# biagiom/spark-network-traffic-classifier

Hardware: NVIDIA H100
Metric: flow-records/sec fit+transform (higher is better)
Workload: dtype u8 bins / uint32 histograms / f64 split scoring (f32 records)

## Files before the change

### spark-network-traffic-classifier_b200/b200flow/forest.py

```python
import math
from dataclasses import dataclass

import numpy as np
import torch

from . import _lib
from ._lib import NODE_DTYPE, SPLIT_DTYPE, B200FlowError, UnsupportedParamError, call, ptr

import os as _os
CHUNK_ROWS = 2048
FUSED = True
TOP_LEVELS = int(_os.environ.get("B200FLOW_TOP_LEVELS", "8"))
DEDUP = True
_PIN = True
PROFILE = None


def _timed(name, fn, *args):
    if PROFILE is None:
        return call(fn, *args)
    e0, e1 = torch.cuda.Event(enable_timing=True), torch.cuda.Event(enable_timing=True)
    e0.record()
    call(fn, *args)
    e1.record()
# ... 552 lines not shown
    if U > 0:
        call("b200flow_bag_fill", ptr(W), T, U, ptr(blk_off), ptr(ent))
    del W, uid

    slot_tree = torch.arange(T, dtype=torch.int32, device=dev)
    slot_nid = torch.ones(T, dtype=torch.int32, device=dev)
    slot_node = torch.arange(T, dtype=torch.int32, device=dev)
    idx = torch.arange(T, dtype=torch.int64, device=dev) * nb
    seg_begin = blk_off[idx].contiguous()
    seg_end = blk_off[idx + nb].contiguous()
    n_slots = T
    level = 0
    per_slot_hist = m * n_bins * C * 4
    group_slots = max(1, HIST_BUDGET_BYTES // per_slot_hist)
    stats = dict(levels=0, slots=0, entries=0, hist_launches=0, rows=n, unique_rows=U)

    stats["route_chunk"], stats["route_passes"] = route_ch if fused else 0, route_passes if fused else 0
    stats["record_format"], stats["record_bytes"] = ("packed", rec_bytes) if field_desc is not None else ("bytes", stride)

    def chunk_table(nch):
        off = torch.empty(nch.shape[0] + 1, dtype=torch.int64, device=dev)
        call("b200flow_exclusive_scan_i32_to_i64", ptr(nch), nch.shape[0], ptr(off), ptr(total))
        return off, int(total.item())

    def level_subsets(ns, s_tree, s_nid):
        sub = torch.empty((ns, m), dtype=torch.int16, device=dev)
        call("b200flow_feature_subsets", seed, ns, ptr(s_tree), ptr(s_nid), F, m, ptr(sub))
        return sub

    def plan_route(ns, split_, begin_, end_, total_out, s_node=None, gain_out=None, cursors_=None):
        nch = torch.empty(ns, dtype=torch.int32, device=dev)
        call("b200flow_plan_route", ns, ptr(split_), ptr(begin_), ptr(end_), route_ch, ptr(s_node), ptr(gain_out), ptr(nch), ptr(cursors_))
        roff = torch.empty(ns + 1, dtype=torch.int64, device=dev)
        call("b200flow_exclusive_scan_i32_to_i64", ptr(nch), ns, ptr(roff), ptr(total_out))
        if PROFILE is not None:
            PROFILE.setdefault("_route_entries", []).append(torch.where(nch > 0, end_ - begin_, torch.zeros_like(end_)).sum())
        return roff

    route_chunks_max = E // route_ch + 1

    world = dist.get_world_size(group) if group is not None else 1
    rank = dist.get_rank(group) if group is not None else 0
    REC = 64 + 12 * C
    use_rs = world > 1 and bdist.is_nccl(group)

    def score_sharded(h_full, gs, sub, lvl, split_, nc_, lc_, rc_):
        K = int(max(1, min(RS_CHUNKS, gs, (gs * hsz * 4) // max(RS_MIN_BYTES, 1))))
        bounds = [gs * i // K for i in range(K + 1)]
        ev0 = None
        if PROFILE is not None:
            ev0 = torch.cuda.Event(enable_timing=True); ev0.record()
        jobs = []
        for k in range(K):
            s0, g = bounds[k], bounds[k + 1] - bounds[k]
            per = -(-g // world)
            mine = torch.empty(per * hsz, dtype=torch.int32, device=dev)
            w = dist.reduce_scatter_tensor(mine, h_full[s0 * hsz:(s0 + world * per) * hsz], group=group, async_op=True)
            jobs.append((s0, g, per, mine, w))
        gathers = []
        for s0, g, per, mine, w in jobs:
            w.wait()
            lo = rank * per
            cnt = max(0, min(per, g - lo))
            local = torch.empty(per * REC, dtype=torch.uint8, device=dev)
            sec = [local[:per * 64], local[per * 64:per * (64 + 4 * C)], local[per * (64 + 4 * C):per * (64 + 8 * C)], local[per * (64 + 8 * C):]]
            if cnt > 0:
                _timed("score_level", "b200flow_score_level", ptr(mine), cnt, ptr(sub[s0 + lo:s0 + lo + cnt]), m, n_bins, C, ptr(feat_bins),
                       ptr(feat_kind), lvl, p.max_depth, int(p.min_instances_per_node), float(p.min_info_gain), ptr(sec[0]), ptr(sec[1]),
                       ptr(sec[2]), ptr(sec[3]))
            gathered = torch.empty((world, per * REC), dtype=torch.uint8, device=dev)
            gw = dist.all_gather_into_tensor(gathered, local, group=group, async_op=True)
            gathers.append((s0, per, gathered, gw))
        for s0, per, gathered, gw in gathers:
            gw.wait()
            o = 0
            for dst, width in ((split_, 64), (nc_.view(torch.uint8), 4 * C), (lc_.view(torch.uint8), 4 * C), (rc_.view(torch.uint8), 4 * C)):
                dst.view(-1)[s0 * width:(s0 + world * per) * width].view(world, per * width).copy_(gathered[:, o:o + per * width])
                o += per * width
        if ev0 is not None:
            ev1 = torch.cuda.Event(enable_timing=True); ev1.record()
            PROFILE.setdefault("level_exchange", []).append((ev0, ev1))

    def run_route(roff, rch_dev, n_parents, split_, child_slot_, cursors_, next_subset_, n_next_cap, route=True):
        hist_next = torch.zeros((n_next_cap + world - 1) * hsz, dtype=torch.int32, device=dev)
        cmax = route_chunks_max + n_parents
        scratch = torch.empty(cmax * 4, dtype=torch.int32, device=dev)
        _timed("route_hist_level", "b200flow_route_hist_level", ptr(rec_tp), rec_stride, F, ptr(field_desc), ptr(ent), ptr(ent2), n_parents,
               ptr(seg_begin), ptr(seg_end), ptr(roff), ptr(rch_dev), cmax, route_ch, ptr(split_), ptr(child_slot_), ptr(cursors_),
               ptr(scratch), ptr(next_subset_), m, n_bins, C, ptr(hist_next), 1 if route else 0)
        _lib.launches += route_passes - 1
        stats["hist_launches"] += route_passes
        return hist_next

    side_stream = torch.cuda.Stream(device=dev)
    host_cnt = torch.empty(5, dtype=torch.int64).pin_memory() if _PIN else None
    subset = level_subsets(n_slots, slot_tree, slot_nid)
    hist_ready = None
    counters = None
    if fused and n_slots * hsz * 4 <= HIST_BUDGET_BYTES:
        pseudo = np.zeros(T, SPLIT_DTYPE); pseudo["bin_thr"] = 255; pseudo["flags"] = 4
        pseudo_t = _lib.h2d(pseudo.view(np.uint8).reshape(T, 64), dev)
        child0 = torch.stack([torch.arange(T, dtype=torch.int32, device=dev),
                              torch.full((T,), -1, dtype=torch.int32, device=dev)], 1).contiguous().view(-1)
        cursors0 = torch.zeros(2 * T, dtype=torch.int32, device=dev)
        roff0 = plan_route(T, pseudo_t, seg_begin, seg_end, total)
        hist_full = run_route(roff0, total, T, pseudo_t, child0, cursors0, subset, T, route=False)
        hist_ready = hist_full[:T * hsz]
    while n_slots > 0:
        grow_pool(pool_size + 2 * n_slots)
        lens = (seg_end - seg_begin) if hist_ready is None else None
        n_alloc = n_slots + world - 1
        split = torch.empty((n_alloc, 64), dtype=torch.uint8, device=dev)
        node_counts = torch.empty((n_alloc, C), dtype=torch.int32, device=dev)
        left_counts = torch.empty((n_alloc, C), dtype=torch.int32, device=dev)
        right_counts = torch.empty((n_alloc, C), dtype=torch.int32, device=dev)
        chunk_off = None
        if hist_ready is None:
            nch = ((lens + (CHUNK_ROWS - 1)) // CHUNK_ROWS).to(torch.int32).contiguous()
            chunk_off, n_chunks = chunk_table(nch)
        groups = [(0, n_slots)] if hist_ready is not None else \
            [(g0, min(n_slots, g0 + group_slots)) for g0 in range(0, n_slots, group_slots)]
        for g0, g1 in groups:
            gs = g1 - g0
            if hist_ready is not None:
                h = hist_ready
            else:
                h = torch.zeros(gs * hsz, dtype=torch.int32, device=dev)
                if g0 == 0 and g1 == n_slots:
                    coff, gch = chunk_off, n_chunks
                else:
                    coff = (chunk_off[g0:g1 + 1] - chunk_off[g0]).contiguous()
                    gch = int((chunk_off[g1] - chunk_off[g0]).item())
                _timed("hist_level", "b200flow_hist_level", ptr(tp), stride, F, ptr(ent), gs,
                       ptr(seg_begin[g0:g1]), ptr(seg_end[g0:g1]), ptr(coff), gch, CHUNK_ROWS, ptr(subset[g0:g1]), m, n_bins, C, ptr(h))
                stats["hist_launches"] += 1
                if PROFILE is not None:
                    PROFILE.setdefault("_hist_entries", []).append(lens[g0:g1].sum())
            if use_rs and hist_ready is not None and gs * hsz * 4 >= RS_MIN_BYTES:
                score_sharded(hist_full, gs, subset, level, split, node_counts, left_counts, right_counts)
                del h
                continue
            if group is not None:
                if PROFILE is not None:
                    ev0 = torch.cuda.Event(enable_timing=True); ev0.record()
                bdist.all_reduce_(h, group)
                if PROFILE is not None:
                    ev1 = torch.cuda.Event(enable_timing=True); ev1.record()
                    PROFILE.setdefault("level_exchange", []).append((ev0, ev1))
            _timed("score_level", "b200flow_score_level", ptr(h), gs, ptr(subset[g0:g1]), m, n_bins, C, ptr(feat_bins), ptr(feat_kind),
                   level, p.max_depth, int(p.min_instances_per_node), float(p.min_info_gain), ptr(split[g0:g1]),
                   ptr(node_counts[g0:g1]), ptr(left_counts[g0:g1]), ptr(right_counts[g0:g1]))
            del h
        split, node_counts, left_counts, right_counts = split[:n_slots], node_counts[:n_slots], left_counts[:n_slots], right_counts[:n_slots]
        hist_ready = None
        nblk = (n_slots + 255) // 256
        if counters is None or counters.numel() < 8 + nblk + 1:
            fresh = torch.zeros(8 + 2 * nblk + 1024, dtype=torch.int64, device=dev)
            if counters is None:
                fresh[0:1].fill_(pool_size)
            else:
                fresh[:8] = counters[:8]
            counters = fresh
        next_tree = torch.empty(2 * n_slots, dtype=torch.int32, device=dev)
        next_nid = torch.empty(2 * n_slots, dtype=torch.int32, device=dev)
        next_node = torch.empty(2 * n_slots, dtype=torch.int32, device=dev)
        next_parent = torch.empty(2 * n_slots, dtype=torch.int32, device=dev)
        child_slot = torch.empty(2 * n_slots, dtype=torch.int32, device=dev)
        _timed("grow_level", "b200flow_grow_level", n_slots, ptr(slot_tree), ptr(slot_nid), ptr(slot_node), ptr(split), ptr(node_counts),
# ... 96 lines not shown
```

### spark-network-traffic-classifier_b200/csrc/forest.cu

```cuda
#include <float.h>
#include <stdlib.h>
#include <string.h>

#include "common.cuh"

namespace b200flow {

constexpr int kMaxSubset = 128;

__global__ void __launch_bounds__(128) feature_subsets_kernel(uint64_t seed, int n_slots, const int32_t* __restrict__ slot_tree,
                                                              const uint32_t* __restrict__ slot_nid, int F, int m,
                                                              uint16_t* subset) {
    int s = blockIdx.x * blockDim.x + threadIdx.x;
    if (s >= n_slots) return;
    uint16_t* out = subset + (int64_t)s * m;
    if (m >= F) { for (int i = 0; i < F; ++i) out[i] = (uint16_t)i; return; }
    uint16_t pos[kMaxSubset], val[kMaxSubset], pick[kMaxSubset];
    int nt = 0;
    const int tree = slot_tree[s]; const uint32_t nid = slot_nid[s];
    uint4 r = make_uint4(0, 0, 0, 0);
    for (int i = 0; i < m; ++i) {
        if ((i & 3) == 0) r = philox_keyed(seed, PURPOSE_FEAT, (uint32_t)tree, nid, (uint32_t)(i >> 2), 0u);
        uint32_t w = (i & 3) == 0 ? r.x : (i & 3) == 1 ? r.y : (i & 3) == 2 ? r.z : r.w;
        int j = i + (int)(w % (uint32_t)(F - i));
// ... 391 lines not shown
    const uint8_t* __restrict__ tp, int stride, const b2f_entry* __restrict__ ent, b2f_entry* ent_out, int n_slots,
    const int64_t* __restrict__ seg_begin, const int64_t* __restrict__ seg_end, const int64_t* __restrict__ chunk_off,
    int chunk_rows, const b200flow_split* __restrict__ split, int32_t* cursors) {
    const int64_t c = blockIdx.x;
    const int s = find_slot(chunk_off, n_slots, c);
    const b200flow_split sp = split[s];
    if (sp.flags & 1) return;
    const bool keepL = !(sp.flags & 2), keepR = !(sp.flags & 4);
    if (!keepL && !keepR) return;
    const int64_t sb = seg_begin[s], se = seg_end[s];
    const int64_t b = sb + (c - chunk_off[s]) * chunk_rows;
    const int64_t e = min(se, b + chunk_rows);
    const int lane = lane_id();
    b2f_entry ents[kPartPerThread]; uint32_t dec = 0;
    int nL = 0, nR = 0;
#pragma unroll
    for (int k = 0; k < kPartPerThread; ++k) {
        const int64_t i = b + threadIdx.x + (int64_t)k * blockDim.x;
        int d = 0; ents[k] = make_uint2(0u, 0u);
        if (i < e) {
            ents[k] = ent[i];
            const int bin = tp[(int64_t)ents[k].x * stride + sp.feat];
            const bool left = sp.kind == 0 ? (bin <= sp.bin_thr) : ((sp.mask[bin >> 6] >> (bin & 63)) & 1ull);
            d = left ? (keepL ? 1 : 0) : (keepR ? 2 : 0);
        }
        dec |= (uint32_t)d << (2 * k);
        nL += __popc(__ballot_sync(0xffffffffu, d == 1));
        nR += __popc(__ballot_sync(0xffffffffu, d == 2));
    }
    int baseL = 0, baseR = 0;
    if (lane == 0) { if (nL) baseL = atomicAdd(&cursors[2 * s], nL); if (nR) baseR = atomicAdd(&cursors[2 * s + 1], nR); }
    baseL = __shfl_sync(0xffffffffu, baseL, 0); baseR = __shfl_sync(0xffffffffu, baseR, 0);
#pragma unroll
    for (int k = 0; k < kPartPerThread; ++k) {
        const int d = (dec >> (2 * k)) & 3;
        const uint32_t mL = __ballot_sync(0xffffffffu, d == 1), mR = __ballot_sync(0xffffffffu, d == 2);
        const uint32_t lt = (1u << lane) - 1u;
        if (d == 1) ent_out[sb + baseL + __popc(mL & lt)] = ents[k];
        else if (d == 2) ent_out[se - 1 - (baseR + __popc(mR & lt))] = ents[k];
        baseL += __popc(mL); baseR += __popc(mR);
    }
}

#ifndef B2F_EVICT_FIRST
#define B2F_EVICT_FIRST 1
#endif
#ifndef B2F_GRAN
#define B2F_GRAN 16
#endif
constexpr int kGran = B2F_GRAN;
__host__ __device__ inline int route_granules(int F) { return (F + 1 + kGran - 1) / kGran; }
__host__ __device__ inline int route_pitch(int F) { return kGran == 16 ? route_granules(F) : (route_granules(F) | 1); }
constexpr bool kEvictFirst = B2F_EVICT_FIRST != 0;

constexpr int kPackedMaxBytes = 64;
__device__ __forceinline__ int packed_swizzle_words(int i, int nq) {
    return nq == 2 ? ((i >> 2) & 1) << 2 : nq == 4 ? ((i >> 1) & 3) << 2 : 0;
}

struct RouteChunk { int32_t slot; int32_t n; long long begin; };

__global__ void route_chunks_kernel(const int64_t* __restrict__ chunk_off, int n_slots, const int64_t* __restrict__ n_chunks_dev,
                                    const int64_t* __restrict__ seg_begin, const int64_t* __restrict__ seg_end, int CH,
                                    RouteChunk* out) {
    int64_t c = (int64_t)blockIdx.x * blockDim.x + threadIdx.x;
    if (c >= *n_chunks_dev) return;
    const int s = find_slot(chunk_off, n_slots, c);
    RouteChunk rc; rc.slot = s; rc.begin = seg_begin[s] + (c - chunk_off[s]) * CH;
    rc.n = (int)(min(seg_end[s], (int64_t)rc.begin + CH) - rc.begin);
    out[c] = rc;
}

struct RouteArgs {
    const uint8_t* tp; int stride; int F;
    const int32_t* field_desc;
    const b2f_entry* ent; b2f_entry* ent_out;
    const RouteChunk* chunks; const int64_t* n_chunks_dev;
    const int64_t* seg_begin; const int64_t* seg_end;
    const b200flow_split* split; const int32_t* child_slot; int32_t* cursors;
    const uint16_t* subset_next; int m_total;
    int j0; int m;
    int n_bins; int C; uint32_t* hist_next;
    int route;
};

__host__ __device__ inline size_t route_tab_bytes(int mp, bool packed) { return packed && mp <= 12 ? (size_t)2 * mp * 32 * 8 : 0; }

template <int M, int NW, int KS, int MERGE, int NQ>
__global__ void __launch_bounds__(NW * 32, NW == 8 ? 3 : (NW == 16 ? 2 : 1)) route_hist_level_kernel(const RouteArgs a) {
    extern __shared__ __align__(16) uint32_t sm_u32[];
    constexpr bool PACKED = NQ > 0;
    constexpr bool kTab = PACKED && M > 0 && MERGE == 2;
    constexpr int kThreads = NW * 32, kSub = KS * 32;
    constexpr int gran = PACKED ? 16 : kGran;
    const int m = M > 0 ? M : a.m;
    const int F = a.F;
    const int tid = threadIdx.x, lane = lane_id(), wid = warp_id();
    const int nq = PACKED ? NQ : route_granules(F);
    const int rs = PACKED ? NQ * 16 : route_pitch(F) * kGran;
    const int nbC = a.n_bins * a.C, hsz = m * nbC;
    const int tile_words = rs * kSub / 4;
    uint32_t* tile = sm_u32 + (size_t)wid * tile_words;
    uint32_t* sh_hist = sm_u32 + (size_t)NW * tile_words;
    int* sh_fpos = (int*)(sh_hist + 2 * hsz);
    uint2* sh_tab = (uint2*)(sh_fpos + 2 * m);
    __shared__ b200flow_split sh_split;
    __shared__ int sh_child[2], sh_route_field;

    const int64_t n_chunks = *a.n_chunks_dev;
    const int64_t c0 = n_chunks * blockIdx.x / gridDim.x, c1 = n_chunks * (blockIdx.x + 1) / gridDim.x;
    if (c0 >= c1) return;
    auto flush = [&]() {
        for (int side = 0; side < 2; ++side) {
            const int cs = sh_child[side];
            if (cs < 0) continue;
            uint32_t* gh = a.hist_next + ((int64_t)cs * a.m_total + a.j0) * nbC;
            uint32_t* sh = sh_hist + side * hsz;
            for (int i = tid; i < hsz; i += kThreads) { const uint32_t v = sh[i]; if (v) { atomicAdd(gh + i, v); sh[i] = 0; } }
        }
    };
    for (int i = tid; i < 2 * hsz; i += kThreads) sh_hist[i] = 0;
    auto desc_at = [&](int64_t c) { return c < c1 ? __ldg((const int4*)(a.chunks + c)) : make_int4(-1, 0, 0, 0); };
    auto count_of = [&](const int4& d) { return min(kSub, d.y - wid * kSub); };
    auto entries_of = [&](const int4& d, b2f_entry* x) {
        const int cn = count_of(d);
        const b2f_entry* ep = a.ent + (((long long)(uint32_t)d.z) | ((long long)d.w << 32)) + wid * kSub;
#pragma unroll
        for (int k = 0; k < KS; ++k) x[k] = lane + 32 * k < cn ? (kEvictFirst ? ld_evict_first_u2(ep + 32 * k + lane) : __ldg(ep + 32 * k + lane)) : make_uint2(0u, 0u);
    };
    constexpr int kNQ = PACKED ? NQ : 1;
    constexpr bool kPow2 = (kNQ & (kNQ - 1)) == 0;
    const int g_e0 = kPow2 ? lane / kNQ : 0, g_q0 = kPow2 ? lane % kNQ : 0;
    const int g_sw = packed_swizzle_words(g_e0, NQ) >> 2;
    const uint8_t* g_src = a.tp + g_q0 * 16;
    uint8_t* g_dst = (uint8_t*)tile + g_e0 * rs + (g_q0 ^ g_sw) * 16;
    const uint32_t inv_nq = (1u << 20) / (uint32_t)nq + 1u;
    auto issue_gather = [&](const int4& d, const b2f_entry* x) {
        const int cn = count_of(d);
        if (PACKED) {
#pragma unroll
            for (int it = 0; it < KS * kNQ; ++it) {
                const int k = it / kNQ;
                if (kPow2) {
                    const int e = it * (32 / kNQ) + g_e0;
                    const uint32_t r = __shfl_sync(0xffffffffu, x[k].x, e & 31);
                    if (e < cn) cp_async16(g_dst + it * 512, g_src + (size_t)r * (kNQ * 16));
                } else {
                    const int c = it * 32 + lane, e = c / kNQ, q = c - e * kNQ;
                    const uint32_t r = __shfl_sync(0xffffffffu, x[k].x, e & 31);
                    if (e < cn) cp_async16((uint8_t*)tile + e * rs + q * 16, a.tp + (size_t)r * (kNQ * 16) + q * 16);
                }
            }
        } else {
            for (int c = lane; c < kSub * nq; c += 32) {
                const int e = (int)(((uint32_t)c * inv_nq) >> 20), q = c - e * nq;
                uint32_t r = __shfl_sync(0xffffffffu, x[0].x, e & 31);
                if (KS == 2) { const uint32_t r1 = __shfl_sync(0xffffffffu, x[KS - 1].x, e & 31); r = e < 32 ? r : r1; }
                if (e < cn) {
                    uint8_t* dst = (uint8_t*)tile + e * rs + q * gran;
                    const uint8_t* src = a.tp + (int64_t)r * a.stride + q * gran;
                    if (gran == 16) cp_async16(dst, src); else if (gran == 8) cp_async8(dst, src); else cp_async4(dst, src);
                }
            }
        }
        cp_async_commit();
    };
    bool pending = false;
    b2f_entry p_e[KS]; uint32_t p_dec = 0; int p_bl = 0, p_br = 0; int64_t p_sb = 0, p_se = 0;
#pragma unroll
    for (int k = 0; k < KS; ++k) p_e[k] = make_uint2(0u, 0u);
    const uint32_t lt = (1u << lane) - 1u;
    auto write_pending = [&]() {
        int baseL = __shfl_sync(0xffffffffu, p_bl, 0), baseR = __shfl_sync(0xffffffffu, p_br, 0);
#pragma unroll
        for (int k = 0; k < KS; ++k) {
            const int d = (p_dec >> (2 * k)) & 3;
            const uint32_t mL = __ballot_sync(0xffffffffu, d == 1), mR = __ballot_sync(0xffffffffu, d == 2);
            if (d == 1) { if (kEvictFirst) st_evict_first_u2(a.ent_out + p_sb + baseL + __popc(mL & lt), p_e[k]); else a.ent_out[p_sb + baseL + __popc(mL & lt)] = p_e[k]; }
            else if (d == 2) { if (kEvictFirst) st_evict_first_u2(a.ent_out + p_se - 1 - (baseR + __popc(mR & lt)), p_e[k]); else a.ent_out[p_se - 1 - (baseR + __popc(mR & lt))] = p_e[k]; }
            baseL += __popc(mL); baseR += __popc(mR);
        }
        pending = false;
    };

    int4 d0 = desc_at(c0), d1 = desc_at(c0 + 1), d2 = desc_at(c0 + 2);
    b2f_entry e[KS], f[KS], g[KS];
    entries_of(d0, e);
    entries_of(d1, f);
    int cur_slot = -1;
    const int lab_pos = PACKED ? __ldg(a.field_desc + F) : F;
    const uint8_t* tile8 = (const uint8_t*)tile;
    auto field = [&](int i, int d) -> uint32_t {
        if (!PACKED) return tile8[d + i * rs];
        const uint32_t v = tile[i * (rs >> 2) + ((d & 0xff) ^ packed_swizzle_words(i, nq))];
        return (v >> ((d >> 8) & 0xff)) & (uint32_t)(d >> 16);
    };
    for (int64_t c = c0; c < c1; ++c) {
        entries_of(d2, g);
        const int4 d3 = desc_at(c + 3);
        issue_gather(d0, e);
        if (pending) write_pending();
        cp_async_wait_all();
        __syncwarp();
        const int s = d0.x;
        if (s != cur_slot) {
            __syncthreads();
            if (cur_slot >= 0) flush();
            __syncthreads();
            if (tid < 16) ((uint32_t*)&sh_split)[tid] = ((const uint32_t*)(a.split + s))[tid];
            if (tid < 2) sh_child[tid] = a.child_slot[2 * s + tid];
            if (tid == 0) { const int fs = max(a.split[s].feat, 0); sh_route_field = PACKED ? a.field_desc[fs] : fs; }
            if (kTab) {
                constexpr int kM = M > 0 ? M : 1;
                for (int idx = tid; idx < 2 * kM * 32; idx += kThreads) {
                    const int side = idx / (kM * 32), t = idx / 32 % kM, ln = idx % 32, j = (ln % kM + t) % kM;
                    const int cs = a.child_slot[2 * s + side];
                    const int fidx = cs >= 0 ? a.subset_next[(int64_t)cs * a.m_total + a.j0 + j] : 0;
                    const uint32_t d = (uint32_t)__ldg(a.field_desc + fidx);
                    const uint32_t word = (d & 0xffu) ^ (uint32_t)packed_swizzle_words(ln, NQ);
                    sh_tab[idx] = make_uint2(word * 4u, ((d >> 8) & 31u) | ((d >> 16) << 8) | ((uint32_t)(side * hsz + j * nbC) << 16));
                }
            } else {
                for (int j = tid; j < 2 * m; j += kThreads) {
                    const int cs = a.child_slot[2 * s + (j >= m)];
                    const int fidx = cs >= 0 ? a.subset_next[(int64_t)cs * a.m_total + a.j0 + (j < m ? j : j - m)] : 0;
                    sh_fpos[j] = PACKED ? a.field_desc[fidx] : fidx;
                }
            }
            cur_slot = s;
            __syncthreads();
        }
        const int cnt = count_of(d0);
        if (cnt > 0) {
            const int cl = sh_child[0], cr = sh_child[1];
            const int fs = sh_route_field, kind = sh_split.kind, thr = sh_split.bin_thr;
            int nL = 0, nR = 0;
            uint32_t dec = 0;
#pragma unroll
            for (int k = 0; k < KS; ++k) {
                const int i = k * 32 + lane;
                int d = 0;
                if (i < cnt) {
                    const int bin = (int)field(i, fs);
                    const bool left = kind == 0 ? (bin <= thr) : ((sh_split.mask[bin >> 6] >> (bin & 63)) & 1ull);
                    d = left ? (cl >= 0 ? 1 : 0) : (cr >= 0 ? 2 : 0);
                }
                dec |= (uint32_t)d << (2 * k);
                const uint32_t mL = __ballot_sync(0xffffffffu, d == 1), mR = __ballot_sync(0xffffffffu, d == 2);
                nL += __popc(mL); nR += __popc(mR);
                if (d != 0) {
                    const uint32_t active = mL | mR;
                    const int side = d - 1;
                    const int* fpos = sh_fpos + side * m;
                    uint32_t* hist = sh_hist + side * hsz;
                    const uint32_t lab = field(i, lab_pos);
                    const uint32_t w = e[k].y;
                    if (M > 0 && MERGE == 1) {
                        const uint32_t tag = (lab << 8) | ((uint32_t)side << 16);
#pragma unroll
                        for (int j = 0; j < M; ++j) {
                            const int fp = fpos[j];
                            const uint32_t bin = field(i, fp);
                            const uint32_t key = bin | tag;
                            uint32_t* addr = &hist[j * nbC + bin * a.C + lab];
                            const int l0 = __ffs(active) - 1;
                            const bool top = key == __shfl_sync(active, key, l0);
                            const uint32_t sum = __reduce_add_sync(active, top ? w : 0u);
                            if (!top || lane == l0) atomicAdd(addr, top ? sum : w);
                        }
                    } else if (kTab) {
                        const uint2* tab = sh_tab + side * (M * 32) + lane;
                        const uint8_t* rec = (const uint8_t*)tile + i * rs;
                        uint32_t* hl = sh_hist + lab;
#pragma unroll
                        for (int t = 0; t < M; ++t) {
                            const uint2 dd = tab[t * 32];
                            const uint32_t v = *(const uint32_t*)(rec + dd.x);
                            const uint32_t bin = __funnelshift_r(v, 0u, dd.y) & ((dd.y >> 8) & 0xffu);
                            atomicAdd(hl + (dd.y >> 16) + bin * a.C, w);
                        }
                    } else if (M > 0 && MERGE == 2) {
                        int j = lane % M;
#pragma unroll
                        for (int t = 0; t < M; ++t) {
                            const int fp = fpos[j];
                            const uint32_t bin = field(i, fp);
                            atomicAdd(&hist[j * nbC + bin * a.C + lab], w);
                            j = j + 1 == M ? 0 : j + 1;
                        }
                    } else {
                        for (int j = 0; j < m; ++j) {
                            const int fp = fpos[j];
                            const uint32_t bin = field(i, fp);
                            atomicAdd(&hist[j * nbC + bin * a.C + lab], w);
                        }
                    }
                }
            }
            __syncwarp();
            if (a.route && (nL | nR)) {
                if (lane == 0) {
                    const unsigned long long old = atomicAdd((unsigned long long*)(a.cursors + 2 * s), (unsigned long long)(uint32_t)nL | ((unsigned long long)(uint32_t)nR << 32));
                    p_bl = (int)(uint32_t)old; p_br = (int)(uint32_t)(old >> 32);
                }
#pragma unroll
                for (int k = 0; k < KS; ++k) p_e[k] = e[k];
                p_dec = dec; p_sb = a.seg_begin[s]; p_se = a.seg_end[s];
                pending = true;
            }
        }
        d0 = d1; d1 = d2; d2 = d3;
#pragma unroll
        for (int k = 0; k < KS; ++k) { e[k] = f[k]; f[k] = g[k]; }
    }
    if (pending) write_pending();
    cp_async_wait_all();
    __syncthreads();
    flush();
}

struct RouteCfg { int nw, ks, m_pass, per_sm; size_t smem; };
constexpr size_t kSmemPerSM = 227 * 1024;
constexpr size_t kSmemCtaOverhead = 1024 + 128;

static size_t route_hist_smem(int rs, bool packed, int mp, int n_bins, int C, int nw, int ks) {
    return (size_t)nw * ks * 32 * rs + 2 * (size_t)mp * n_bins * C * 4 + 2 * (size_t)mp * 4 + route_tab_bytes(mp, packed) + 64;
}
static int route_max_ctas(int nw) { return nw == 8 ? 3 : (nw == 16 ? 2 : 1); }

static bool route_cfg(int F, int rs, bool packed, int m, int n_bins, int C, RouteCfg* out) {
    static const int cand[5][2] = {{8, 2}, {8, 1}, {16, 2}, {16, 1}, {32, 1}};
    int force_nw = 0, force_ks = 0;
    { const char* e = getenv("B200FLOW_ROUTE_SHAPE"); if (e && sscanf(e, "%dx%d", &force_nw, &force_ks) != 2) force_nw = force_ks = 0; }
    if (F <= 0 || F > 255 || m <= 0 || n_bins <= 0 || C <= 0) return false;
    auto fits = [&](int mp, int nw, int ks) { return route_hist_smem(rs, packed, mp, n_bins, C, nw, ks) + kSmemCtaOverhead <= kSmemPerSM; };
    int mp = m;
    while (mp >= 1 && !fits(mp, 8, 1)) --mp;
    if (mp < 1) return false;
    const int passes = (m + mp - 1) / mp;
    mp = (m + passes - 1) / passes;
    int best = -1; long best_key = -1;
    for (int i = 0; i < 5; ++i) {
        const int nw = cand[i][0], ks = cand[i][1];
        if (force_nw > 0 && (nw != force_nw || ks != force_ks)) continue;
        if (!fits(mp, nw, ks)) continue;
        const size_t smem = route_hist_smem(rs, packed, mp, n_bins, C, nw, ks);
        int per_sm = (int)(kSmemPerSM / (smem + kSmemCtaOverhead));
        if (per_sm > route_max_ctas(nw)) per_sm = route_max_ctas(nw);
        const int warps = per_sm * nw > 32 ? 32 : per_sm * nw;
        const long key = ((long)(warps * ks < 48 ? warps * ks : 48) << 20) + ((long)(1023 - nw * ks) << 10) + warps;
        if (key > best_key) { best_key = key; best = i; }
    }
    if (best < 0) return false;
    out->nw = cand[best][0]; out->ks = cand[best][1]; out->m_pass = mp;
    out->smem = route_hist_smem(rs, packed, mp, n_bins, C, out->nw, out->ks);
    out->per_sm = (int)(kSmemPerSM / (out->smem + kSmemCtaOverhead));
    if (out->per_sm > route_max_ctas(out->nw)) out->per_sm = route_max_ctas(out->nw);
    return true;
}

static int route_hist_variant() {
    const char* e = getenv("B200FLOW_ROUTE_VARIANT");
    if (e && !strcmp(e, "merge")) return 1;
    if (e && !strcmp(e, "generic")) return 0;
    return 2;
}

template <int NW, int KS, int NQ>
static cudaError_t route_launch(int M, int merge, unsigned grid_cap, size_t smem, int per_sm_hint, int waves, int64_t n_chunks_max,
                                const RouteArgs& a, cudaStream_t st) {
    cudaError_t e = cudaSuccess;
#define B2F_ROUTE_GO(KERNEL)                                                                                                   \
    {                                                                                                                          \
        e = cudaFuncSetAttribute(KERNEL, cudaFuncAttributeMaxDynamicSharedMemorySize, (int)smem);                             \
        if (e != cudaSuccess) return e;                                                                                        \
        int per_sm = 0;                                                                                                        \
        e = cudaOccupancyMaxActiveBlocksPerMultiprocessor(&per_sm, KERNEL, NW * 32, smem);                                    \
        if (e != cudaSuccess) return e;                                                                                        \
        if (per_sm < 1) per_sm = per_sm_hint > 0 ? per_sm_hint : 1;                                                            \
        const int64_t want = (int64_t)kNumSMs * per_sm * waves;                                                                \
        unsigned grid = (unsigned)(n_chunks_max < want ? n_chunks_max : want);                                                 \
        if (grid_cap && grid > grid_cap) grid = grid_cap;                                                                      \
        KERNEL<<<grid, NW * 32, smem, st>>>(a);                                                                                \
    }
#define B2F_ROUTE_CASE(MM)                                                                                                     \
    case MM:                                                                                                                   \
        if (merge == 1) B2F_ROUTE_GO((route_hist_level_kernel<MM, NW, KS, 1, NQ>))                                         \
        else if (merge == 2) B2F_ROUTE_GO((route_hist_level_kernel<MM, NW, KS, 2, NQ>))                                    \
        else B2F_ROUTE_GO((route_hist_level_kernel<0, NW, KS, 0, NQ>))                                                     \
        break;
    switch (M) {
        B2F_ROUTE_CASE(1) B2F_ROUTE_CASE(2) B2F_ROUTE_CASE(3) B2F_ROUTE_CASE(4) B2F_ROUTE_CASE(5) B2F_ROUTE_CASE(6)
        B2F_ROUTE_CASE(7) B2F_ROUTE_CASE(8) B2F_ROUTE_CASE(9) B2F_ROUTE_CASE(10) B2F_ROUTE_CASE(11) B2F_ROUTE_CASE(12)
        default: B2F_ROUTE_GO((route_hist_level_kernel<0, NW, KS, 0, NQ>)) break;
    }
#undef B2F_ROUTE_CASE
#undef B2F_ROUTE_GO
    return cudaGetLastError();
}

template <int NQ>
static cudaError_t route_shape(const RouteCfg& cfg, int M, int merge, size_t smem, int waves, int64_t n_chunks_max, const RouteArgs& a,
                               cudaStream_t st) {
    if (cfg.nw == 8 && cfg.ks == 2) return route_launch<8, 2, NQ>(M, merge, 0, smem, cfg.per_sm, waves, n_chunks_max, a, st);
    if (cfg.nw == 8) return route_launch<8, 1, NQ>(M, merge, 0, smem, cfg.per_sm, waves, n_chunks_max, a, st);
    if (cfg.nw == 16 && cfg.ks == 2) return route_launch<16, 2, NQ>(M, merge, 0, smem, cfg.per_sm, waves, n_chunks_max, a, st);
    if (cfg.nw == 16) return route_launch<16, 1, NQ>(M, merge, 0, smem, cfg.per_sm, waves, n_chunks_max, a, st);
    return route_launch<32, 1, NQ>(M, merge, 0, smem, cfg.per_sm, waves, n_chunks_max, a, st);
}

__global__ void next_segments_kernel(int n_next, const int64_t* __restrict__ n_next_dev, const int32_t* __restrict__ next_parent,
                                     const int64_t* __restrict__ seg_begin, const int64_t* __restrict__ seg_end,
                                     const int32_t* __restrict__ cursors, int64_t* next_begin, int64_t* next_end) {
    int i = blockIdx.x * blockDim.x + threadIdx.x;
    if (i >= n_next || (n_next_dev && i >= *n_next_dev)) return;
    const int p = next_parent[i], ps = p >> 1;
    if ((p & 1) == 0) { next_begin[i] = seg_begin[ps]; next_end[i] = seg_begin[ps] + cursors[2 * ps]; }
    else { next_begin[i] = seg_end[ps] - cursors[2 * ps + 1]; next_end[i] = seg_end[ps]; }
}

__global__ void finalize_forest_kernel(int64_t n_nodes, const uint32_t* __restrict__ pool_counts, int C, double* leaf_prob) {
    int64_t i = (int64_t)blockIdx.x * blockDim.x + threadIdx.x;
    if (i >= n_nodes) return;
    double tot = 0.0;
    for (int k = 0; k < C; ++k) tot += (double)pool_counts[i * C + k];
    for (int k = 0; k < C; ++k) leaf_prob[i * C + k] = tot != 0.0 ? (double)pool_counts[i * C + k] / tot : 0.0;
}

}

using namespace b200flow;

extern "C" int b200flow_feature_subsets(uint64_t seed, int32_t n_slots, const int32_t* slot_tree, const uint32_t* slot_nid,
                                        int32_t F, int32_t m, uint16_t* subset, void* stream) {
    B2F_REQUIRE(slot_tree && slot_nid && subset && F > 0 && F < 65536 && m > 0 && m <= F, "feature_subsets: bad arguments");
    B2F_REQUIRE(m == F || m <= kMaxSubset, "feature_subsets: subset size %d > %d not supported", m, kMaxSubset);
    if (n_slots <= 0) return B200FLOW_OK;
    feature_subsets_kernel<<<(n_slots + 127) / 128, 128, 0, (cudaStream_t)stream>>>(seed, n_slots, slot_tree, slot_nid, F, m, subset);
    return check_launch("feature_subsets");
}
// ... 84 lines not shown
                                      const int64_t* seg_end, const int32_t* cursors, int64_t* next_begin, int64_t* next_end, void* stream) {
    B2F_REQUIRE(next_parent && seg_begin && seg_end && cursors && next_begin && next_end, "next_segments: null pointer");
    if (n_next <= 0) return B200FLOW_OK;
    next_segments_kernel<<<(n_next + 255) / 256, 256, 0, (cudaStream_t)stream>>>(n_next, n_next_dev, next_parent, seg_begin, seg_end, cursors, next_begin, next_end);
    return check_launch("next_segments");
}

extern "C" int b200flow_finalize_forest(int64_t n_nodes, const uint32_t* pool_counts, int32_t C, double* leaf_prob, void* stream) {
    B2F_REQUIRE(pool_counts && leaf_prob && C > 0, "finalize_forest: bad arguments");
    if (n_nodes <= 0) return B200FLOW_OK;
    finalize_forest_kernel<<<(unsigned)((n_nodes + 255) / 256), 256, 0, (cudaStream_t)stream>>>(n_nodes, pool_counts, C, leaf_prob);
    return check_launch("finalize_forest");
}

extern "C" int b200flow_packed_layout(int32_t F, const int32_t* feat_bins, int32_t C, int32_t* desc, int32_t* rec_bytes) {
    B2F_REQUIRE(feat_bins && desc && rec_bytes && F > 0 && C > 0 && C <= 256, "packed_layout: bad arguments");
    *rec_bytes = 0;
    if (F > 255) return B200FLOW_OK;
    int width[256], order[256], used[256];
    auto bits = [](int v) { int b = 0; while (v > 0) { ++b; v >>= 1; } return b > 0 ? b : 1; };
    for (int f = 0; f <= F; ++f) {
        const int nb = f < F ? feat_bins[f] : C;
        B2F_REQUIRE(nb >= 1 && nb <= 256, "packed_layout: field %d has %d values", f, nb);
        width[f] = bits(nb - 1);
        order[f] = f;
    }
    for (int i = 1; i <= F; ++i) {
        const int f = order[i]; int k = i - 1;
        while (k >= 0 && width[order[k]] < width[f]) { order[k + 1] = order[k]; --k; }
        order[k + 1] = f;
    }
    int nw = 0;
    for (int i = 0; i <= F; ++i) {
        const int f = order[i];
        int w = 0;
        while (w < nw && used[w] + width[f] > 32) ++w;
        if (w == nw) used[nw++] = 0;
        desc[f] = w | (used[w] << 8) | (((1 << width[f]) - 1) << 16);
        used[w] += width[f];
    }
    const int bytes = (nw * 4 + 15) / 16 * 16;
    *rec_bytes = bytes <= kPackedMaxBytes && bytes + 16 <= route_pitch(F) * kGran ? bytes : 0;
    return B200FLOW_OK;
}

extern "C" int b200flow_route_hist_config(int32_t F, int32_t m, int32_t n_bins, int32_t C, int32_t rec_bytes, int32_t* chunk_rows,
                                          int32_t* m_pass) {
    RouteCfg cfg;
    if (rec_bytes < 0 || !route_cfg(F, rec_bytes > 0 ? rec_bytes : route_pitch(F) * kGran, rec_bytes > 0, m, n_bins, C, &cfg)) return 0;
    if (chunk_rows) *chunk_rows = cfg.nw * cfg.ks * 32;
    if (m_pass) *m_pass = cfg.m_pass;
    return 1;
}

extern "C" int b200flow_route_hist_level(const uint8_t* tp, int32_t tp_stride, int32_t F, const int32_t* field_desc,
                                         const void* ent, void* ent_out,
                                         int32_t n_slots, const int64_t* seg_begin, const int64_t* seg_end, const int64_t* chunk_off,
                                         const int64_t* n_chunks_dev, int64_t n_chunks_max, int32_t chunk_rows,
                                         const b200flow_split* split, const int32_t* child_slot,
                                         int32_t* cursors, void* chunk_scratch, const uint16_t* subset_next, int32_t m, int32_t n_bins,
                                         int32_t C, uint32_t* hist_next, int32_t flags, void* stream) {
    B2F_REQUIRE(tp && ent && seg_begin && seg_end && chunk_off && n_chunks_dev && split && child_slot && chunk_scratch &&
                    subset_next && hist_next, "route_hist_level: null pointer");
    const bool route = (flags & 1) != 0;
    B2F_REQUIRE(!route || (ent_out && cursors && ((uintptr_t)cursors & 7) == 0), "route_hist_level: routing needs ent_out and 8-byte aligned cursors");
    if (field_desc)
        B2F_REQUIRE((tp_stride & 15) == 0 && tp_stride > 0 && tp_stride <= kPackedMaxBytes && ((uintptr_t)tp & 15) == 0,
                    "route_hist_level: packed records must be 16-byte multiples up to %d bytes, 16-byte aligned", kPackedMaxBytes);
    else
        B2F_REQUIRE((tp_stride & 15) == 0 && tp_stride >= (F + 1 + 15) / 16 * 16 && ((uintptr_t)tp & 15) == 0, "route_hist_level: bad TreePoint stride/alignment");
    B2F_REQUIRE(((uintptr_t)chunk_scratch & 15) == 0, "route_hist_level: chunk_scratch must be 16-byte aligned");
    RouteCfg cfg;
    const int rs = field_desc ? tp_stride : route_pitch(F) * kGran;
    B2F_REQUIRE(route_cfg(F, rs, field_desc != nullptr, m, n_bins, C, &cfg), "route_hist_level: one feature's child histograms exceed shared memory (use partition_level + hist_level)");
    B2F_REQUIRE(chunk_rows == cfg.nw * cfg.ks * 32, "route_hist_level: chunk_rows must be the value of b200flow_route_hist_config (%d)", cfg.nw * cfg.ks * 32);
    if (n_slots <= 0 || n_chunks_max <= 0) return B200FLOW_OK;
    cudaStream_t st = (cudaStream_t)stream;
    RouteChunk* chunks = (RouteChunk*)chunk_scratch;
    route_chunks_kernel<<<(unsigned)((n_chunks_max + 255) / 256), 256, 0, st>>>(chunk_off, n_slots, n_chunks_dev, seg_begin,
                                                                             seg_end, chunk_rows, chunks);
    RouteArgs a;
    a.tp = tp; a.stride = tp_stride; a.F = F; a.field_desc = field_desc; a.ent = (const b2f_entry*)ent; a.ent_out = (b2f_entry*)ent_out; a.chunks = chunks; a.n_chunks_dev = n_chunks_dev;
    a.seg_begin = seg_begin; a.seg_end = seg_end; a.split = split; a.child_slot = child_slot; a.cursors = cursors;
    a.subset_next = subset_next; a.m_total = m; a.n_bins = n_bins; a.C = C; a.hist_next = hist_next;
    static int waves = -1;
    if (waves < 0) { const char* e = getenv("B200FLOW_ROUTE_WAVES"); waves = e ? atoi(e) : 2; if (waves < 1) waves = 1; }
    int merge = route_hist_variant();
    if (merge == 1 && C > 128) merge = 2;
    for (int j0 = 0, pass = 0; j0 < m; j0 += cfg.m_pass, ++pass) {
        a.j0 = j0; a.m = m - j0 < cfg.m_pass ? m - j0 : cfg.m_pass; a.route = (route && pass == 0) ? 1 : 0;
        const int M = a.m <= 12 ? a.m : 0;
        const size_t smem = route_hist_smem(rs, field_desc != nullptr, a.m, n_bins, C, cfg.nw, cfg.ks);
        cudaError_t e;
        switch (field_desc ? tp_stride / 16 : 0) {
            case 1: e = route_shape<1>(cfg, M, merge, smem, waves, n_chunks_max, a, st); break;
            case 2: e = route_shape<2>(cfg, M, merge, smem, waves, n_chunks_max, a, st); break;
            case 3: e = route_shape<3>(cfg, M, merge, smem, waves, n_chunks_max, a, st); break;
            case 4: e = route_shape<4>(cfg, M, merge, smem, waves, n_chunks_max, a, st); break;
            default: e = route_shape<0>(cfg, M, merge, smem, waves, n_chunks_max, a, st); break;
        }
        if (e != cudaSuccess) { set_error("route_hist_level: %s", cudaGetErrorString(e)); return B200FLOW_ERR_CUDA; }
    }
    return check_launch("route_hist_level");
}
```

Before: 156.2 million.

## Double-buffer per-slot route headers and feature tables in route_hist kernel

Moves the per-slot split, child slots, route field and feature-position/lookup tables into a shared-memory header array with up to two sets. When shared memory allows it without lowering CTAs per SM, the next chunk's slot tables are built ahead of time so a slot change only swaps buffers instead of rebuilding behind extra barriers. This aims to cut the serialized setup and __syncthreads cost at slot boundaries, at the price of more shared memory and extra build work per chunk. Profiling hooks for histogram zeroing are also added.

After: 157.4 million (median of 6 runs). Within noise of the previous version (+0.8%).

```diff
diff --git a/spark-network-traffic-classifier_b200/b200flow/forest.py b/spark-network-traffic-classifier_b200/b200flow/forest.py
--- a/spark-network-traffic-classifier_b200/b200flow/forest.py
+++ b/spark-network-traffic-classifier_b200/b200flow/forest.py
@@ -658,8 +658,14 @@
             PROFILE.setdefault("level_exchange", []).append((ev0, ev1))
 
     def run_route(roff, rch_dev, n_parents, split_, child_slot_, cursors_, next_subset_, n_next_cap, route=True):
+        if PROFILE is not None:
+            z0 = torch.cuda.Event(enable_timing=True); z0.record()
         hist_next = torch.zeros((n_next_cap + world - 1) * hsz, dtype=torch.int32, device=dev)
         cmax = route_chunks_max + n_parents
+        if PROFILE is not None:
+            z1 = torch.cuda.Event(enable_timing=True); z1.record()
+            PROFILE.setdefault("_hist_zero", []).append((z0, z1, hist_next.numel() * 4))
+            PROFILE.setdefault("_route_plan", []).append((roff, n_parents, cmax, route_ch))
         scratch = torch.empty(cmax * 4, dtype=torch.int32, device=dev)
         _timed("route_hist_level", "b200flow_route_hist_level", ptr(rec_tp), rec_stride, F, ptr(field_desc), ptr(ent), ptr(ent2), n_parents,
                ptr(seg_begin), ptr(seg_end), ptr(roff), ptr(rch_dev), cmax, route_ch, ptr(split_), ptr(child_slot_), ptr(cursors_),
diff --git a/spark-network-traffic-classifier_b200/csrc/forest.cu b/spark-network-traffic-classifier_b200/csrc/forest.cu
--- a/spark-network-traffic-classifier_b200/csrc/forest.cu
+++ b/spark-network-traffic-classifier_b200/csrc/forest.cu
@@ -497,7 +497,10 @@
     int j0; int m;
     int n_bins; int C; uint32_t* hist_next;
     int route;
+    int sets;
 };
+
+struct RouteSlotHdr { b200flow_split split; int child[2]; int route_field; int pad; };
 
 __host__ __device__ inline size_t route_tab_bytes(int mp, bool packed) { return packed && mp <= 12 ? (size_t)2 * mp * 32 * 8 : 0; }
 
@@ -518,16 +521,16 @@
     uint32_t* tile = sm_u32 + (size_t)wid * tile_words;
     uint32_t* sh_hist = sm_u32 + (size_t)NW * tile_words;
     int* sh_fpos = (int*)(sh_hist + 2 * hsz);
-    uint2* sh_tab = (uint2*)(sh_fpos + 2 * m);
-    __shared__ b200flow_split sh_split;
-    __shared__ int sh_child[2], sh_route_field;
+    uint2* sh_tab = (uint2*)(sh_fpos + a.sets * 2 * m);
+    RouteSlotHdr* sh_hdr = (RouteSlotHdr*)((uint8_t*)sh_tab + a.sets * route_tab_bytes(m, PACKED));
+    int cur = 0;
 
     const int64_t n_chunks = *a.n_chunks_dev;
     const int64_t c0 = n_chunks * blockIdx.x / gridDim.x, c1 = n_chunks * (blockIdx.x + 1) / gridDim.x;
     if (c0 >= c1) return;
     auto flush = [&]() {
         for (int side = 0; side < 2; ++side) {
-            const int cs = sh_child[side];
+            const int cs = sh_hdr[cur].child[side];
             if (cs < 0) continue;
             uint32_t* gh = a.hist_next + ((int64_t)cs * a.m_total + a.j0) * nbC;
             uint32_t* sh = sh_hist + side * hsz;
@@ -598,11 +601,38 @@
         pending = false;
     };
 
+    auto build = [&](int set, int s) {
+        RouteSlotHdr* h = sh_hdr + set;
+        if (tid < 16) ((uint32_t*)&h->split)[tid] = ((const uint32_t*)(a.split + s))[tid];
+        if (tid < 2) h->child[tid] = a.child_slot[2 * s + tid];
+        if (tid == 0) { const int fs = max(a.split[s].feat, 0); h->route_field = PACKED ? a.field_desc[fs] : fs; }
+        if (kTab) {
+            constexpr int kM = M > 0 ? M : 1;
+            uint2* tab = sh_tab + set * (2 * kM * 32);
+            for (int idx = tid; idx < 2 * kM * 32; idx += kThreads) {
+                const int side = idx / (kM * 32), t = idx / 32 % kM, ln = idx % 32, j = (ln % kM + t) % kM;
+                const int cs = a.child_slot[2 * s + side];
+                const int fidx = cs >= 0 ? a.subset_next[(int64_t)cs * a.m_total + a.j0 + j] : 0;
+                const uint32_t d = (uint32_t)__ldg(a.field_desc + fidx);
+                const uint32_t word = (d & 0xffu) ^ (uint32_t)packed_swizzle_words(ln, NQ);
+                tab[idx] = make_uint2(word * 4u, ((d >> 8) & 31u) | ((d >> 16) << 8) | ((uint32_t)(side * hsz + j * nbC) << 16));
+            }
+        } else {
+            int* fpos = sh_fpos + set * 2 * m;
+            for (int j = tid; j < 2 * m; j += kThreads) {
+                const int cs = a.child_slot[2 * s + (j >= m)];
+                const int fidx = cs >= 0 ? a.subset_next[(int64_t)cs * a.m_total + a.j0 + (j < m ? j : j - m)] : 0;
+                fpos[j] = PACKED ? a.field_desc[fidx] : fidx;
+            }
+        }
+    };
     int4 d0 = desc_at(c0), d1 = desc_at(c0 + 1), d2 = desc_at(c0 + 2);
     b2f_entry e[KS], f[KS], g[KS];
     entries_of(d0, e);
     entries_of(d1, f);
-    int cur_slot = -1;
+    build(0, d0.x);
+    int cur_slot = d0.x;
+    __syncthreads();
     const int lab_pos = PACKED ? __ldg(a.field_desc + F) : F;
     const uint8_t* tile8 = (const uint8_t*)tile;
     auto field = [&](int i, int d) -> uint32_t {
@@ -614,41 +644,31 @@
         entries_of(d2, g);
         const int4 d3 = desc_at(c + 3);
         issue_gather(d0, e);
+        const int s = d0.x;
+        const bool change = s != cur_slot;
+        const bool ahead = a.sets == 2 && d1.x >= 0 && d1.x != s;
+        if (ahead && !change) build(cur ^ 1, d1.x);
         if (pending) write_pending();
         cp_async_wait_all();
         __syncwarp();
-        const int s = d0.x;
-        if (s != cur_slot) {
+        if (change) {
             __syncthreads();
-            if (cur_slot >= 0) flush();
+            flush();
             __syncthreads();
-            if (tid < 16) ((uint32_t*)&sh_split)[tid] = ((const uint32_t*)(a.split + s))[tid];
-            if (tid < 2) sh_child[tid] = a.child_slot[2 * s + tid];
-            if (tid == 0) { const int fs = max(a.split[s].feat, 0); sh_route_field = PACKED ? a.field_desc[fs] : fs; }
-            if (kTab) {
-                constexpr int kM = M > 0 ? M : 1;
-                for (int idx = tid; idx < 2 * kM * 32; idx += kThreads) {
-                    const int side = idx / (kM * 32), t = idx / 32 % kM, ln = idx % 32, j = (ln % kM + t) % kM;
-                    const int cs = a.child_slot[2 * s + side];
-                    const int fidx = cs >= 0 ? a.subset_next[(int64_t)cs * a.m_total + a.j0 + j] : 0;
-                    const uint32_t d = (uint32_t)__ldg(a.field_desc + fidx);
-                    const uint32_t word = (d & 0xffu) ^ (uint32_t)packed_swizzle_words(ln, NQ);
-                    sh_tab[idx] = make_uint2(word * 4u, ((d >> 8) & 31u) | ((d >> 16) << 8) | ((uint32_t)(side * hsz + j * nbC) << 16));
-                }
+            if (a.sets == 2) {
+                cur ^= 1;
             } else {
-                for (int j = tid; j < 2 * m; j += kThreads) {
-                    const int cs = a.child_slot[2 * s + (j >= m)];
-                    const int fidx = cs >= 0 ? a.subset_next[(int64_t)cs * a.m_total + a.j0 + (j < m ? j : j - m)] : 0;
-                    sh_fpos[j] = PACKED ? a.field_desc[fidx] : fidx;
-                }
+                build(0, s);
+                __syncthreads();
             }
             cur_slot = s;
-            __syncthreads();
+            if (ahead) build(cur ^ 1, d1.x);
         }
         const int cnt = count_of(d0);
         if (cnt > 0) {
-            const int cl = sh_child[0], cr = sh_child[1];
-            const int fs = sh_route_field, kind = sh_split.kind, thr = sh_split.bin_thr;
+            const RouteSlotHdr& hd = sh_hdr[cur];
+            const int cl = hd.child[0], cr = hd.child[1];
+            const int fs = hd.route_field, kind = hd.split.kind, thr = hd.split.bin_thr;
             int nL = 0, nR = 0;
             uint32_t dec = 0;
 #pragma unroll
@@ -657,7 +677,7 @@
                 int d = 0;
                 if (i < cnt) {
                     const int bin = (int)field(i, fs);
-                    const bool left = kind == 0 ? (bin <= thr) : ((sh_split.mask[bin >> 6] >> (bin & 63)) & 1ull);
+                    const bool left = kind == 0 ? (bin <= thr) : ((hd.split.mask[bin >> 6] >> (bin & 63)) & 1ull);
                     d = left ? (cl >= 0 ? 1 : 0) : (cr >= 0 ? 2 : 0);
                 }
                 dec |= (uint32_t)d << (2 * k);
@@ -666,7 +686,7 @@
                 if (d != 0) {
                     const uint32_t active = mL | mR;
                     const int side = d - 1;
-                    const int* fpos = sh_fpos + side * m;
+                    const int* fpos = sh_fpos + (cur * 2 + side) * m;
                     uint32_t* hist = sh_hist + side * hsz;
                     const uint32_t lab = field(i, lab_pos);
                     const uint32_t w = e[k].y;
@@ -684,7 +704,7 @@
                             if (!top || lane == l0) atomicAdd(addr, top ? sum : w);
                         }
                     } else if (kTab) {
-                        const uint2* tab = sh_tab + side * (M * 32) + lane;
+                        const uint2* tab = sh_tab + (cur * 2 + side) * (M * 32) + lane;
                         const uint8_t* rec = (const uint8_t*)tile + i * rs;
                         uint32_t* hl = sh_hist + lab;
 #pragma unroll
@@ -734,12 +754,13 @@
     flush();
 }
 
-struct RouteCfg { int nw, ks, m_pass, per_sm; size_t smem; };
+struct RouteCfg { int nw, ks, m_pass, per_sm, sets; size_t smem; };
 constexpr size_t kSmemPerSM = 227 * 1024;
 constexpr size_t kSmemCtaOverhead = 1024 + 128;
 
-static size_t route_hist_smem(int rs, bool packed, int mp, int n_bins, int C, int nw, int ks) {
-    return (size_t)nw * ks * 32 * rs + 2 * (size_t)mp * n_bins * C * 4 + 2 * (size_t)mp * 4 + route_tab_bytes(mp, packed) + 64;
+static size_t route_hist_smem(int rs, bool packed, int mp, int n_bins, int C, int nw, int ks, int sets) {
+    return (size_t)nw * ks * 32 * rs + 2 * (size_t)mp * n_bins * C * 4 +
+           (size_t)sets * (2 * (size_t)mp * 4 + route_tab_bytes(mp, packed) + sizeof(RouteSlotHdr)) + 64;
 }
 static int route_max_ctas(int nw) { return nw == 8 ? 3 : (nw == 16 ? 2 : 1); }
 
@@ -748,7 +769,7 @@
     int force_nw = 0, force_ks = 0;
     { const char* e = getenv("B200FLOW_ROUTE_SHAPE"); if (e && sscanf(e, "%dx%d", &force_nw, &force_ks) != 2) force_nw = force_ks = 0; }
     if (F <= 0 || F > 255 || m <= 0 || n_bins <= 0 || C <= 0) return false;
-    auto fits = [&](int mp, int nw, int ks) { return route_hist_smem(rs, packed, mp, n_bins, C, nw, ks) + kSmemCtaOverhead <= kSmemPerSM; };
+    auto fits = [&](int mp, int nw, int ks) { return route_hist_smem(rs, packed, mp, n_bins, C, nw, ks, 1) + kSmemCtaOverhead <= kSmemPerSM; };
     int mp = m;
     while (mp >= 1 && !fits(mp, 8, 1)) --mp;
     if (mp < 1) return false;
@@ -759,7 +780,7 @@
         const int nw = cand[i][0], ks = cand[i][1];
         if (force_nw > 0 && (nw != force_nw || ks != force_ks)) continue;
         if (!fits(mp, nw, ks)) continue;
-        const size_t smem = route_hist_smem(rs, packed, mp, n_bins, C, nw, ks);
+        const size_t smem = route_hist_smem(rs, packed, mp, n_bins, C, nw, ks, 1);
         int per_sm = (int)(kSmemPerSM / (smem + kSmemCtaOverhead));
         if (per_sm > route_max_ctas(nw)) per_sm = route_max_ctas(nw);
         const int warps = per_sm * nw > 32 ? 32 : per_sm * nw;
@@ -768,9 +789,13 @@
     }
     if (best < 0) return false;
     out->nw = cand[best][0]; out->ks = cand[best][1]; out->m_pass = mp;
-    out->smem = route_hist_smem(rs, packed, mp, n_bins, C, out->nw, out->ks);
-    out->per_sm = (int)(kSmemPerSM / (out->smem + kSmemCtaOverhead));
-    if (out->per_sm > route_max_ctas(out->nw)) out->per_sm = route_max_ctas(out->nw);
+    auto per_sm_of = [&](int sets) {
+        const int p = (int)(kSmemPerSM / (route_hist_smem(rs, packed, mp, n_bins, C, out->nw, out->ks, sets) + kSmemCtaOverhead));
+        return p < route_max_ctas(out->nw) ? p : route_max_ctas(out->nw);
+    };
+    out->per_sm = per_sm_of(1);
+    out->sets = per_sm_of(2) == out->per_sm ? 2 : 1;
+    out->smem = route_hist_smem(rs, packed, mp, n_bins, C, out->nw, out->ks, out->sets);
     return true;
 }
 
@@ -1021,7 +1046,7 @@
     RouteArgs a;
     a.tp = tp; a.stride = tp_stride; a.F = F; a.field_desc = field_desc; a.ent = (const b2f_entry*)ent; a.ent_out = (b2f_entry*)ent_out; a.chunks = chunks; a.n_chunks_dev = n_chunks_dev;
     a.seg_begin = seg_begin; a.seg_end = seg_end; a.split = split; a.child_slot = child_slot; a.cursors = cursors;
-    a.subset_next = subset_next; a.m_total = m; a.n_bins = n_bins; a.C = C; a.hist_next = hist_next;
+    a.subset_next = subset_next; a.m_total = m; a.n_bins = n_bins; a.C = C; a.hist_next = hist_next; a.sets = cfg.sets;
     static int waves = -1;
     if (waves < 0) { const char* e = getenv("B200FLOW_ROUTE_WAVES"); waves = e ? atoi(e) : 2; if (waves < 1) waves = 1; }
     int merge = route_hist_variant();
@@ -1029,7 +1054,7 @@
     for (int j0 = 0, pass = 0; j0 < m; j0 += cfg.m_pass, ++pass) {
         a.j0 = j0; a.m = m - j0 < cfg.m_pass ? m - j0 : cfg.m_pass; a.route = (route && pass == 0) ? 1 : 0;
         const int M = a.m <= 12 ? a.m : 0;
-        const size_t smem = route_hist_smem(rs, field_desc != nullptr, a.m, n_bins, C, cfg.nw, cfg.ks);
+        const size_t smem = route_hist_smem(rs, field_desc != nullptr, a.m, n_bins, C, cfg.nw, cfg.ks, cfg.sets);
         cudaError_t e;
         switch (field_desc ? tp_stride / 16 : 0) {
             case 1: e = route_shape<1>(cfg, M, merge, smem, waves, n_chunks_max, a, st); break;
```
